# yumi-crew/pose_estimation

Hardware: NVIDIA B200
Metric: icp_hypotheses_per_s (higher is better)
Workload: dtype f32

## Files before the change

### pose_estimation_b200/csrc/icp.cu

```cuda
#include <algorithm>

#include "block_select.cuh"
#include "nn_cache.cuh"
#include "nn_graph.cuh"
#include "nn_search.cuh"
#include "nn_upfront.cuh"

namespace peb {

namespace {

constexpr int kIcpThreads = 128;
constexpr int kMinBlocksSingle = 5;
#ifndef PEB_MIN_BLOCKS_BATCH
#define PEB_MIN_BLOCKS_BATCH 8
#endif
constexpr int kMinBlocksBatch = PEB_MIN_BLOCKS_BATCH;
#ifndef PEB_MIN_BLOCKS_SEARCH
#define PEB_MIN_BLOCKS_SEARCH 10
#endif
constexpr int kMinBlocksSearch = PEB_MIN_BLOCKS_SEARCH;

struct IcpLaunch {
  GridView grid;
// ... 111 lines not shown
    sm[warp][lane] = v;
  }
  __syncthreads();
  if (threadIdx.x < NACC) {
    double r = 0.0;
#pragma unroll
    for (int w = 0; w < kW; ++w) r += sm[w][threadIdx.x];
    sm_out[threadIdx.x] = r;
  }
  __syncthreads();
}

__global__ void __launch_bounds__(128) icp_anchor_kernel(const IcpLaunch L, int* __restrict__ anchors) {
  const int a = blockIdx.x * blockDim.x + threadIdx.x;
  const int h = blockIdx.y;
  if (a >= L.n_anchor) return;
  const IcpState* st = L.states + h;
  float T[16];
  bool apply = false;
#pragma unroll
  for (int i = 0; i < 16; ++i) {
    T[i] = __ldcg(&st->final_t.m[i]);
    if (T[i] != ((i % 5 == 0) ? 1.0f : 0.0f)) apply = true;
  }
  float4 p = L.src[32 * a];
  if (apply) {
    float ox, oy, oz;
    transform_icp(T, p.x, p.y, p.z, ox, oy, oz);
    p.x = ox;
    p.y = oy;
    p.z = oz;
  }
  const NnBest best = grid_nn<1, true>(L.grid, p.x, p.y, p.z, L.stop_d2);
  anchors[static_cast<size_t>(h) * L.n_anchor + a] = best.j;
}

__device__ __forceinline__ unsigned long long global_ns() {
  unsigned long long t;
  asm volatile("mov.u64 %0, %%globaltimer;" : "=l"(t));
  return t;
}

template <int MB>
__device__ __noinline__ void finish_iteration(IcpState* st, const IcpCriteria* cr, const double* acc, Mat4* trace,
                                              int trace_cap, unsigned long long* dbg) {
  if (dbg) dbg[5] = global_ns();
  IcpState s = *st;
  if (dbg) dbg[6] = global_ns() + (s.iterations < -5 ? 1 : 0);
  icp_finish_iteration(s, *cr, acc);
  if (dbg) dbg[7] = global_ns() + (s.iterations < -5 ? 1 : 0);
  s.ticket = 0;
  if (trace && s.state != PEB_NO_CORRESPONDENCES && s.iterations >= 1 && s.iterations <= trace_cap)
    trace[s.iterations - 1] = s.inc;
  *st = s;
}

__device__ __forceinline__ void pdl_trigger_and_wait() {
  asm volatile("griddepcontrol.launch_dependents;");
  asm volatile("griddepcontrol.wait;" ::: "memory");
}

__device__ __forceinline__ int ld_acquire_gpu(const int* p) {
  int v;
  asm volatile("ld.acquire.gpu.global.s32 %0, [%1];" : "=r"(v) : "l"(p) : "memory");
  return v;
}


constexpr int kEpochStopped = 1 << 20;
constexpr unsigned long long kFlagWaitLimitNs = 20ull * 1000ull * 1000ull * 1000ull;
__device__ __forceinline__ void wait_for_hypothesis(const int* __restrict__ solved, int need, int* err_flag) {
  if (threadIdx.x == 0 && ld_acquire_gpu(solved) < need) {
    const unsigned long long t0 = global_ns();
    unsigned spins = 0;
    while (ld_acquire_gpu(solved) < need) {
      __nanosleep(40);
      if ((++spins & 0xFFFu) == 0u && global_ns() - t0 > kFlagWaitLimitNs) {
        atomicExch(err_flag, 1);
        break;
      }
    }
  }
  __syncthreads();
}

__device__ __forceinline__ void wait_for_search(const int* __restrict__ searched, int need, const int* __restrict__ solved,
                                                int* err_flag) {
  if (threadIdx.x == 0 && ld_acquire_gpu(searched) < need && ld_acquire_gpu(solved) < kEpochStopped) {
    const unsigned long long t0 = global_ns();
    unsigned spins = 0;
    while (ld_acquire_gpu(searched) < need && ld_acquire_gpu(solved) < kEpochStopped) {
      __nanosleep(40);
      if ((++spins & 0xFFFu) == 0u && global_ns() - t0 > kFlagWaitLimitNs) {
        atomicExch(err_flag, 1);
        break;
      }
    }
  }
  __syncthreads();
}

__device__ __forceinline__ bool graph_pays(const IcpLaunch& L, const IcpState* st) {
  if (!L.knn) return false;
  if (L.knn_kappa <= 0.0f) return true;
  const double mse = __ldcg(&st->cur_mse);
  const double cnt = __ldcg(L.knn_stat + 1);
  return cnt > 0.0 && 4.0 * mse * static_cast<double>(L.knn_kappa) * cnt < __ldcg(L.knn_stat);
}

template <int EST, int NACC>
__device__ __forceinline__ void accumulate_pair_impl(const GridView& g, const float4& p, const NnBest& best,
                                                     double (&acc)[NACC]) {
  const float4 t = g.pts[best.j];
  if (EST == PEB_ESTIMATOR_SVD) {
    const double sx = p.x, sy = p.y, sz = p.z, tx = t.x, ty = t.y, tz = t.z;
    acc[0] += 1.0;
    acc[1] += sx;
    acc[2] += sy;
    acc[3] += sz;
    acc[4] += tx;
    acc[5] += ty;
    acc[6] += tz;
    acc[7] = fma(tx, sx, acc[7]);
    acc[8] = fma(tx, sy, acc[8]);
    acc[9] = fma(tx, sz, acc[9]);
    acc[10] = fma(ty, sx, acc[10]);
    acc[11] = fma(ty, sy, acc[11]);
    acc[12] = fma(ty, sz, acc[12]);
    acc[13] = fma(tz, sx, acc[13]);
    acc[14] = fma(tz, sy, acc[14]);
    acc[15] = fma(tz, sz, acc[15]);
    acc[16] += static_cast<double>(best.d2);
  } else {
    acc[0] += 1.0;
    acc[NACC - 1] += static_cast<double>(best.d2);
    const float4 nr = g.normals[best.j];
    if (finite3(t.x, t.y, t.z) && finite3(nr.x, nr.y, nr.z)) {
      const float sx = p.x, sy = p.y, sz = p.z, dx = t.x, dy = t.y, dz = t.z;
      const float nx = nr.x, ny = nr.y, nz = nr.z;
      const double a = nz * sy - ny * sz;
      const double b = nx * sz - nz * sx;
      const double c = ny * sx - nx * sy;
      acc[1] += a * a;
      acc[2] += a * b;
      acc[3] += a * c;
      acc[4] += a * nx;
      acc[5] += a * ny;
      acc[6] += a * nz;
      acc[7] += b * b;
      acc[8] += b * c;
      acc[9] += b * nx;
      acc[10] += b * ny;
      acc[11] += b * nz;
      acc[12] += c * c;
      acc[13] += c * nx;
      acc[14] += c * ny;
      acc[15] += c * nz;
      acc[16] += nx * nx;
      acc[17] += nx * ny;
      acc[18] += nx * nz;
      acc[19] += ny * ny;
      acc[20] += ny * nz;
      acc[21] += nz * nz;
      const double d = nx * dx + ny * dy + nz * dz - nx * sx - ny * sy - nz * sz;
      acc[22] += a * d;
      acc[23] += b * d;
      acc[24] += c * d;
      acc[25] += nx * d;
      acc[26] += ny * d;
      acc[27] += nz * d;
    }
  }
}
template <int EST, int NACC>
__device__ __forceinline__ void accumulate_pair(const GridView& g, const float4& p, const NnBest& best,
                                                double (&acc)[NACC]) {
  static_assert((EST == PEB_ESTIMATOR_SVD && NACC == kAccSvd) || (EST != PEB_ESTIMATOR_SVD && NACC == kAccLls), "layout");
  accumulate_pair_impl<EST, NACC>(g, p, best, acc);
}

__device__ __forceinline__ NnBest first_iteration_search(const IcpLaunch& L, int h, int i, bool valid, const float4& p,
                                                         const float* T, bool apply, CoopTile* tile) {
  NnBest best;
  best.d2 = pos_inf();
  best.idx = -1;
  best.j = -1;
  bool need = false;
  int group = 0;
  if (valid) {
    int j_seed = -1;
    float4 a = make_float4(0.f, 0.f, 0.f, 0.f);
    group = 0;
    const int patch = i >> 5;
#pragma unroll 1
    for (int k = 0; k < 2 && j_seed < 0; ++k) {
      const int pa = patch + k;
      if (pa >= L.n_anchor) break;
      const int js = __ldcg(L.anchors + static_cast<size_t>(h) * L.n_anchor + pa);
      if (js < 0) continue;
      a = L.src[32 * pa];
      if (apply) {
        float ox, oy, oz;
        transform_icp(T, a.x, a.y, a.z, ox, oy, oz);
        a.x = ox;
        a.y = oy;
        a.z = oz;
      }
      const float ax = p.x - a.x, ay = p.y - a.y, az = p.z - a.z;
      if (ax * ax + ay * ay + az * az <= L.seed_guard2 * L.grid.h * L.grid.h) {
        j_seed = js;
        group = k;
      }
    }
    if (j_seed >= 0) {
      best = (L.knn && L.cold_graph) ? grid_nn_graph_descend(L.grid, L.knn, p.x, p.y, p.z, j_seed)
                                     : grid_nn_seed_probe(L.grid, p.x, p.y, p.z, j_seed, a.x, a.y, a.z);
      need = true;
    } else {
      best = grid_nn<1>(L.grid, p.x, p.y, p.z, L.stop_d2);
      PEB_COOP_COUNT_LANE(6);
    }
  }
  PEB_COOP_COUNT(7, __any_sync(0xFFFFFFFFu, valid && !need) ? 1 : 0);
#pragma unroll 1
  for (int k = 0; k < 2; ++k) {
    const bool mine = need && group == k;
    bool done = false;
    if (L.coop_max_rows > 0) done = grid_nn_coop_verify(L.grid, tile, mine, p.x, p.y, p.z, L.stop_d2, L.coop_max_rows, best);
    if (!done && mine) grid_ball_search(L.grid, p.x, p.y, p.z, L.stop_d2, best);
  }
  return best;
}

template <int G, int EST, bool CERT, int UPF, int NACC>
__device__ __forceinline__ void icp_query(const IcpLaunch& L, const int h, float4* __restrict__ work, const int i,
                                          const bool first, const bool apply, const bool graph, const float* T,
                                          CoopTile* tile, double (&acc)[NACC]) {
  const int lane_in_group = threadIdx.x & (G - 1);
  const bool in = i < L.n_src;
  float4 p = make_float4(0.f, 0.f, 0.f, 1.f);
  if (in) p = first ? L.src[i] : work[i];
  const int j_prev = first ? -1 : __float_as_int(p.w);
  const bool valid = in && finite3(p.x, p.y, p.z);
  float moved = 0.0f;
  if (valid && apply) {
    float ox, oy, oz;
    transform_icp(T, p.x, p.y, p.z, ox, oy, oz);
    if (CERT) {
      const float mx = ox - p.x, my = oy - p.y, mz = oz - p.z;
      moved = sqrtf(mx * mx + my * my + mz * mz);
    }
    p.x = ox;
    p.y = oy;
    p.z = oz;
  }
  NnBest best;
  best.d2 = pos_inf();
  best.idx = -1;
  best.j = -1;
  float slack = -1.0f;
  if (G == 1 && first && L.anchors) {
    best = first_iteration_search(L, h, i, valid, p, T, apply, tile);
    if (CERT && valid) L.slack[static_cast<size_t>(h) * L.n_src + i] = -1.0f;
  } else if (valid) {
    float* sl = L.slack + static_cast<size_t>(h) * L.n_src + i;
    if (G == 1 && L.warm && j_prev >= 0 && j_prev < L.grid.n) {
      if (CERT) {
        slack = *sl - 2.000002f * moved - 1e-5f * L.grid.h;
        if (slack > 0.0f) {
          const float4 t = L.grid.pts[j_prev];
          best.d2 = l2_simple(p.x, p.y, p.z, t.x, t.y, t.z);
          best.idx = __float_as_int(t.w);
          best.j = j_prev;
        } else {
          best = grid_nn_warm_cert(L.grid, p.x, p.y, p.z, j_prev, L.stop_d2, L.margin, &slack);
        }
        *sl = slack;
      } else {
        if (UPF == 4 || UPF == 6) best = graph ? grid_nn_warm_graph(L.grid, L.knn, p.x, p.y, p.z, j_prev, L.stop_d2, kGraphSkipHopeless, L.launch_idx <= L.knn_peek_until, UPF == 6 ? L.knn_aux : nullptr)
                                   : grid_nn_warm(L.grid, p.x, p.y, p.z, j_prev, L.stop_d2);
        else best = UPF ? grid_nn_warm_upfront<(UPF == 3 ? 3 : 2)>(L.grid, p.x, p.y, p.z, j_prev, L.stop_d2)
                        : grid_nn_warm(L.grid, p.x, p.y, p.z, j_prev, L.stop_d2);
      }
    } else {
      best = grid_nn<G>(L.grid, p.x, p.y, p.z, L.stop_d2);
      if (CERT && lane_in_group == 0) *sl = -1.0f;
    }
  }
  if (in && lane_in_group == 0 && (first || valid)) {
    p.w = __int_as_float(best.j);
    work[i] = p;
  }
  bool keep = valid && best.idx >= 0;
  if (keep && static_cast<double>(best.d2) > L.max_dist_sqr) keep = false;
  if (keep && L.use_rejector && !(best.d2 < L.rej_max2)) keep = false;
  if (in && lane_in_group == 0 && L.corr_idx) {
    const int orig = __float_as_int(L.src[i].w);
    L.corr_idx[orig] = keep ? best.idx : -1;
    L.corr_d2[orig] = keep ? best.d2 : 0.0f;
  }
  if (keep && lane_in_group == 0) accumulate_pair<EST>(L.grid, p, best, acc);
}

template <int UPF>
__device__ __forceinline__ NnBest icp_search_query(const IcpLaunch& L, const int h, float4* __restrict__ work, const int i,
                                                   const bool first, const bool apply, const bool graph, const float* T,
                                                   CoopTile* tile, float4& p, bool& valid) {
  const bool in = i < L.n_src;
  p = make_float4(0.f, 0.f, 0.f, 1.f);
  if (in) p = first ? L.src[i] : work[i];
  const int j_prev = first ? -1 : __float_as_int(p.w);
  valid = in && finite3(p.x, p.y, p.z);
  if (valid && apply) {
    float ox, oy, oz;
    transform_icp(T, p.x, p.y, p.z, ox, oy, oz);
    p.x = ox;
    p.y = oy;
    p.z = oz;
  }
  NnBest best;
  best.d2 = pos_inf();
  best.idx = -1;
  best.j = -1;
  if (first && L.anchors) {
    best = first_iteration_search(L, h, i, valid, p, T, apply, tile);
  } else if (valid) {
    if (L.warm && j_prev >= 0 && j_prev < L.grid.n) {
      if (UPF == 4 || UPF == 6) best = graph ? grid_nn_warm_graph(L.grid, L.knn, p.x, p.y, p.z, j_prev, L.stop_d2, kGraphSkipHopeless, L.launch_idx <= L.knn_peek_until, UPF == 6 ? L.knn_aux : nullptr)
                                 : grid_nn_warm(L.grid, p.x, p.y, p.z, j_prev, L.stop_d2);
      else best = grid_nn_warm(L.grid, p.x, p.y, p.z, j_prev, L.stop_d2);
    } else {
      best = grid_nn<1>(L.grid, p.x, p.y, p.z, L.stop_d2);
    }
  }
  if (in && (first || valid)) {
    p.w = __int_as_float(best.j);
    work[i] = p;
  }
  return best;
}

__device__ __forceinline__ bool keep_pair(const IcpLaunch& L, const bool valid, const NnBest& best) {
  bool keep = valid && best.idx >= 0;
  if (keep && static_cast<double>(best.d2) > L.max_dist_sqr) keep = false;
  if (keep && L.use_rejector && !(best.d2 < L.rej_max2)) keep = false;
  return keep;
}

template <bool FIRST, int UPF>
__device__ __forceinline__ void load_launch_flags(const IcpLaunch& L, const IcpState* st, float* s_inc, int* s_flags) {
  if (threadIdx.x < 16) s_inc[threadIdx.x] = FIRST ? __ldcg(&st->final_t.m[threadIdx.x]) : __ldcg(&st->inc.m[threadIdx.x]);
  if (threadIdx.x == 32) {
    const int active = __ldcg(&st->active);
    const int first = FIRST ? 1 : 0;
    int apply = 1;
    if (first) {
      apply = 0;
      for (int i = 0; i < 16; ++i) {
        const float g = __ldcg(&st->final_t.m[i]);
        if (g != ((i % 5 == 0) ? 1.0f : 0.0f)) apply = 1;
      }
    }
    s_flags[0] = active;
    s_flags[1] = first;
    s_flags[2] = apply;
    const int graph = ((UPF == 4 || UPF == 6) && graph_pays(L, st)) ? 1 : 0;
    s_flags[3] = graph;
  }
}

template <int G, int EST, int MB, bool CERT, bool FIRST, int UPF>
__device__ __forceinline__ void icp_iteration_body(const IcpLaunch& L, const int h, const int blk) {
  unsigned long long t_dbg[5];
  if (L.dbg) t_dbg[0] = global_ns();
  constexpr int NACC = (EST == PEB_ESTIMATOR_SVD) ? kAccSvd : kAccLls;
  __shared__ double sm[kIcpThreads / 32][kAccMax];
  __shared__ double sm_tot[kAccMax];
  __shared__ float s_inc[16];
  __shared__ int s_flags[4];
  __shared__ CoopTile s_tile[kIcpThreads / 32];
  IcpState* st = L.states + h;
  if (threadIdx.x < 16) s_inc[threadIdx.x] = FIRST ? __ldcg(&st->final_t.m[threadIdx.x]) : __ldcg(&st->inc.m[threadIdx.x]);
  if (threadIdx.x == 32) {
    const int active = __ldcg(&st->active);
    const int first = FIRST ? 1 : 0;
    int apply = 1;
    if (first) {
      apply = 0;
      for (int i = 0; i < 16; ++i) {
        const float g = __ldcg(&st->final_t.m[i]);
        if (g != ((i % 5 == 0) ? 1.0f : 0.0f)) apply = 1;
      }
    }
    s_flags[0] = active;
    s_flags[1] = first;
    s_flags[2] = apply;
    const int graph = ((UPF == 4 || UPF == 6) && graph_pays(L, st)) ? 1 : 0;
    s_flags[3] = graph;
  }
  __syncthreads();
  if (!s_flags[0]) return;
  constexpr bool first = FIRST;
  const bool apply = s_flags[2] != 0;
  const float* T = s_inc;

  double acc[NACC];
#pragma unroll
  for (int i = 0; i < NACC; ++i) acc[i] = 0.0;

  float4* work = L.work + static_cast<size_t>(h) * L.n_src;
  constexpr int kQ = kIcpThreads / G;
  const int q_local = threadIdx.x / G;
  const bool graph = (UPF == 4 || UPF == 6) && s_flags[3] != 0;
  for (int base = blk * kQ; base < L.n_src; base += L.blocks_per_hyp * kQ)
    icp_query<G, EST, CERT, UPF>(L, h, work, base + q_local, first, apply, graph, T, &s_tile[threadIdx.x >> 5], acc);

  if (L.dbg) t_dbg[1] = global_ns();
  const double r = block_reduce_acc<NACC>(acc, sm);
  double* part = L.partials + (static_cast<size_t>(h) * L.part_stride) * kAccMax;
  if (threadIdx.x < NACC) __stcg(part + static_cast<size_t>(blk) * kAccMax + threadIdx.x, r);
  __threadfence();
  __syncthreads();
  __shared__ int s_last;
  if (threadIdx.x == 0) {
    const unsigned t = atomicAdd(&st->ticket, 1u);
    s_last = (t == static_cast<unsigned>(L.blocks_per_hyp) - 1u);
  }
  __syncthreads();
  if (!s_last) return;
  __threadfence();
  if (L.dbg) t_dbg[2] = global_ns();
  reduce_partials<NACC>(part, L.blocks_per_hyp, sm, sm_tot);
  if (L.dbg) t_dbg[3] = global_ns();
  if (threadIdx.x == 0) {
    finish_iteration<MB>(st, &L.crit, sm_tot, L.trace, L.trace_cap, (L.dbg && h == 0) ? L.dbg + 8 * L.launch_idx : nullptr);
    if (L.dbg && h == 0) {
      t_dbg[4] = global_ns();
      for (int k = 0; k < 5; ++k) L.dbg[8 * L.launch_idx + k] = t_dbg[k];
    }
    if (L.epochs) {
      const int still_active = st->active;
      __threadfence();
      atomicAdd(L.epochs + h, still_active ? 1 : kEpochStopped);
    }
  }
}

template <int G, int EST, int MB, bool CERT, bool FIRST, int UPF = 0>
__global__ void __launch_bounds__(kIcpThreads, MB) icp_iteration_kernel(const IcpLaunch L) {
  if (FIRST || L.epochs == nullptr) {
    pdl_trigger_and_wait();
  } else {
    asm volatile("griddepcontrol.launch_dependents;");
    wait_for_hypothesis(L.epochs + blockIdx.y, L.launch_idx, L.err_flag);
  }
  icp_iteration_body<G, EST, MB, CERT, FIRST, UPF>(L, blockIdx.y, blockIdx.x);
}

template <int MB, bool FIRST, int UPF>
__global__ void __launch_bounds__(kIcpThreads, MB) icp_search_kernel(const IcpLaunch L) {
  if (FIRST || L.epochs == nullptr) {
    pdl_trigger_and_wait();
  } else {
    asm volatile("griddepcontrol.launch_dependents;");
    wait_for_hypothesis(L.epochs + blockIdx.y, L.launch_idx, L.err_flag);
  }
  const int h = blockIdx.y, blk = blockIdx.x;
  __shared__ float s_inc[16];
  __shared__ int s_flags[4];
  __shared__ CoopTile s_tile[kIcpThreads / 32];
  IcpState* st = L.states + h;
  load_launch_flags<FIRST, UPF>(L, st, s_inc, s_flags);
  __syncthreads();
  if (s_flags[0]) {
    const bool apply = s_flags[2] != 0;
    const bool graph = (UPF == 4 || UPF == 6) && s_flags[3] != 0;
    float4* work = L.work + static_cast<size_t>(h) * L.n_src;
    for (int base = blk * kIcpThreads; base < L.n_src; base += gridDim.x * kIcpThreads) {
      const int i = base + threadIdx.x;
      float4 p;
      bool valid;
      const NnBest best = icp_search_query<UPF>(L, h, work, i, FIRST, apply, graph, s_inc, &s_tile[threadIdx.x >> 5], p, valid);
      int* w = reinterpret_cast<int*>(work + i) + 3;
      if (valid && best.j >= 0 && !finite3(p.x, p.y, p.z)) *w = -2 - best.j;
      else if (!FIRST && !valid && i < L.n_src && __float_as_int(p.w) <= -2) *w = -1;
    }
  }
  if (L.epochs && s_flags[0]) {
    __syncthreads();
    if (threadIdx.x == 0) {
      __threadfence();
      if (atomicAdd(&st->ticket_search, 1u) == gridDim.x - 1u) {
        st->ticket_search = 0u;
        __threadfence();
        atomicAdd(&st->searched, 1);
      }
    }
  }
}

template <int EST, int MB, bool CHAIN>
__global__ void __launch_bounds__(kIcpThreads, MB) icp_moment_kernel(const IcpLaunch L, const unsigned char* __restrict__ kept) {
  if (L.epochs == nullptr) {
    pdl_trigger_and_wait();
  } else {
    asm volatile("griddepcontrol.launch_dependents;");
    wait_for_search(&L.states[blockIdx.y].searched, L.launch_idx + 1, L.epochs + blockIdx.y, L.err_flag);
  }
  const int h = blockIdx.y, blk = blockIdx.x;
  constexpr int NACC = (EST == PEB_ESTIMATOR_SVD) ? kAccSvd : kAccLls;
  __shared__ double sm[kIcpThreads / 32][kAccMax];
  __shared__ double sm_tot[kAccMax];
  __shared__ int s_active;
  IcpState* st = L.states + h;
  if (threadIdx.x == 0) s_active = __ldcg(&st->active);
  __syncthreads();
  if (!s_active) return;

  double acc[NACC];
#pragma unroll
  for (int i = 0; i < NACC; ++i) acc[i] = 0.0;
  const float4* work = L.work + static_cast<size_t>(h) * L.n_src;
  for (int i = blk * kIcpThreads + threadIdx.x; i < L.n_src; i += L.blocks_per_hyp * kIcpThreads) {
    const float4 p = __ldcg(work + i);
    bool valid = finite3(p.x, p.y, p.z);
    int j = __float_as_int(p.w);
    if (j <= -2) {
      valid = true;
      j = -2 - j;
    }
    if (CHAIN) {
      NnBest best;
      const bool keep = valid && j >= 0 && kept[static_cast<size_t>(h) * L.n_src + i];
      if (keep) {
        const float4 t = L.grid.pts[j];
        best.d2 = l2_simple(p.x, p.y, p.z, t.x, t.y, t.z);
        best.idx = point_index(t);
        best.j = j;
        accumulate_pair<EST>(L.grid, p, best, acc);
      }
      if (L.corr_idx) {
        const int orig = __float_as_int(L.src[i].w);
        L.corr_idx[orig] = keep ? best.idx : -1;
        L.corr_d2[orig] = keep ? best.d2 : 0.0f;
      }
      continue;
    }
    if (!valid || j < 0) continue;
    const float4 t = L.grid.pts[j];
    NnBest best;
    best.d2 = l2_simple(p.x, p.y, p.z, t.x, t.y, t.z);
    best.idx = point_index(t);
    best.j = j;
    if (keep_pair(L, valid, best)) accumulate_pair<EST>(L.grid, p, best, acc);
  }

  const double r = block_reduce_acc<NACC>(acc, sm);
  double* part = L.partials + (static_cast<size_t>(h) * L.part_stride) * kAccMax;
  if (threadIdx.x < NACC) __stcg(part + static_cast<size_t>(blk) * kAccMax + threadIdx.x, r);
  __threadfence();
  __syncthreads();
  __shared__ int s_last;
  if (threadIdx.x == 0) {
    const unsigned t = atomicAdd(&st->ticket, 1u);
    s_last = (t == static_cast<unsigned>(L.blocks_per_hyp) - 1u);
  }
  __syncthreads();
  if (!s_last) return;
  __threadfence();
  reduce_partials<NACC>(part, L.blocks_per_hyp, sm, sm_tot);
  if (threadIdx.x == 0) {
    finish_iteration<MB>(st, &L.crit, sm_tot, L.trace, L.trace_cap, nullptr);
    if (L.epochs) {
      const int still_active = st->active;
      __threadfence();
      atomicAdd(L.epochs + h, still_active ? 1 : kEpochStopped);
    }
  }
}

constexpr int kRejThreads = 1024;

struct RejChain {
  int kind[PEB_MAX_REJECTORS];
  int min_corr[PEB_MAX_REJECTORS];
  double value[PEB_MAX_REJECTORS];
  int n;
  unsigned char* kept;
  unsigned long long* o2o;
};

__device__ __forceinline__ NnBest rej_pair(const IcpLaunch& L, const float4* __restrict__ work, int i, float4& p, bool& valid) {
  p = __ldcg(work + i);
  valid = finite3(p.x, p.y, p.z);
  int j = __float_as_int(p.w);
  if (j <= -2) {
    valid = true;
    j = -2 - j;
  }
  NnBest best;
  best.d2 = pos_inf();
  best.idx = -1;
  best.j = -1;
  if (valid && j >= 0) {
    const float4 t = L.grid.pts[j];
    best.d2 = l2_simple(p.x, p.y, p.z, t.x, t.y, t.z);
    best.idx = point_index(t);
    best.j = j;
  }
  return best;
}

__device__ __forceinline__ unsigned abs_bits(float v) { return __float_as_uint(v) & 0x7FFFFFFFu; }

__device__ __forceinline__ float rej_score(const IcpLaunch& L, const float4& p, int j) {
  const float4 t = L.grid.pts[j];
  const float dx = p.x - t.x, dy = p.y - t.y, dz = p.z - t.z;
  return __fadd_rn(__fadd_rn(__fmul_rn(dx, dx), __fmul_rn(dz, dz)), __fmul_rn(dy, dy));
}

__device__ __forceinline__ int rej_count(const unsigned char* kept, int n) {
  int m = 0;
  for (int base = 0; base < n; base += kRejThreads) {
    const int i = base + threadIdx.x;
    m += __syncthreads_count(i < n && kept[i]);
  }
  return m;
}

__global__ void __launch_bounds__(kRejThreads, 1) icp_reject_kernel(const IcpLaunch L, const RejChain R) {
  pdl_trigger_and_wait();
  __shared__ unsigned hist[2048];
  __shared__ unsigned s_state[2];
  __shared__ unsigned s_wsum[32];
  __shared__ int s_active;
  const int h = blockIdx.x;
  if (threadIdx.x == 0) s_active = __ldcg(&L.states[h].active);
  __syncthreads();
  if (!s_active) return;
  const int n = L.n_src;
  const float4* work = L.work + static_cast<size_t>(h) * n;
  unsigned char* kept = R.kept + static_cast<size_t>(h) * n;
  unsigned long long* tab = R.o2o ? R.o2o + static_cast<size_t>(h) * L.grid.n : nullptr;
  for (int i = threadIdx.x; i < n; i += kRejThreads) {
    float4 p;
    bool valid;
    const NnBest b = rej_pair(L, work, i, p, valid);
    kept[i] = keep_pair(L, valid, b) ? 1 : 0;
  }
  __syncthreads();
  for (int s = 0; s < R.n; ++s) {
    const int kind = R.kind[s];
    if (kind == PEB_REJECTOR_DISTANCE) {
      const float lim = static_cast<float>(R.value[s] * R.value[s]);
      for (int i = threadIdx.x; i < n; i += kRejThreads) {
        if (!kept[i]) continue;
        float4 p;
        bool valid;
        const NnBest b = rej_pair(L, work, i, p, valid);
        if (!(b.d2 < lim)) kept[i] = 0;
      }
    } else if (kind == PEB_REJECTOR_MEDIAN_DISTANCE) {
      const int m = rej_count(kept, n);
      if (m == 0) continue;
      auto score = [&](int i) {
        if (!kept[i]) return -1.0f;
        float4 p;
        bool valid;
        const NnBest b = rej_pair(L, work, i, p, valid);
        return __uint_as_float(abs_bits(rej_score(L, p, b.j)));
      };
      const float med = block_select_nth<decltype(score), true>(score, n, m / 2, hist, s_state, s_wsum);
      const double lim = static_cast<double>(med) * R.value[s];
      for (int i = threadIdx.x; i < n; i += kRejThreads) {
        if (!kept[i]) continue;
        float4 p;
        bool valid;
        const NnBest b = rej_pair(L, work, i, p, valid);
        if (!(static_cast<double>(rej_score(L, p, b.j)) <= lim)) kept[i] = 0;
      }
    } else if (kind == PEB_REJECTOR_ONE_TO_ONE) {
      for (int i = threadIdx.x; i < n; i += kRejThreads) {
        if (!kept[i]) continue;
        float4 p;
        bool valid;
        const NnBest b = rej_pair(L, work, i, p, valid);
        const unsigned long long key = (static_cast<unsigned long long>(abs_bits(b.d2)) << 32) |
                                       static_cast<unsigned>(__float_as_int(L.src[i].w));
        atomicMin(tab + b.j, key);
      }
      __syncthreads();
      for (int i = threadIdx.x; i < n; i += kRejThreads) {
        if (!kept[i]) continue;
        float4 p;
        bool valid;
        const NnBest b = rej_pair(L, work, i, p, valid);
        const unsigned long long key = (static_cast<unsigned long long>(abs_bits(b.d2)) << 32) |
                                       static_cast<unsigned>(__float_as_int(L.src[i].w));
        if (__ldcg(tab + b.j) == key) __stcg(tab + b.j, ~0ull);
        else kept[i] = 0;
      }
    } else {
      const int m = rej_count(kept, n);
      const float ratio = fminf(1.0f, fmaxf(0.0f, static_cast<float>(R.value[s])));
      const int n_keep = max(static_cast<int>(floorf(ratio * static_cast<float>(m))), R.min_corr[s]);
      if (n_keep >= m) continue;
      unsigned vb = 0u;
      int o_cut = -1;
      if (n_keep > 0) {
        auto d2_of = [&](int i) {
          if (!kept[i]) return -1.0f;
          float4 p;
          bool valid;
          return __uint_as_float(abs_bits(rej_pair(L, work, i, p, valid).d2));
        };
        vb = __float_as_uint(block_select_nth<decltype(d2_of), true>(d2_of, n, n_keep - 1, hist, s_state, s_wsum));
        int below = 0;
        for (int base = 0; base < n; base += kRejThreads) {
          const int i = base + threadIdx.x;
          bool lt = false;
          if (i < n && kept[i]) {
            float4 p;
            bool valid;
            lt = abs_bits(rej_pair(L, work, i, p, valid).d2) < vb;
          }
          below += __syncthreads_count(lt);
        }
        auto src_at_cut = [&](int i) {
          if (!kept[i]) return -1.0f;
          float4 p;
          bool valid;
          if (abs_bits(rej_pair(L, work, i, p, valid).d2) != vb) return -1.0f;
          return __int_as_float(__float_as_int(L.src[i].w));
        };
        o_cut = __float_as_int(block_select_nth<decltype(src_at_cut), true>(src_at_cut, n, n_keep - below - 1, hist, s_state, s_wsum));
      }
      for (int i = threadIdx.x; i < n; i += kRejThreads) {
        if (!kept[i]) continue;
        bool stay = false;
        if (n_keep > 0) {
          float4 p;
          bool valid;
          const unsigned db = abs_bits(rej_pair(L, work, i, p, valid).d2);
          stay = db < vb || (db == vb && __float_as_int(L.src[i].w) <= o_cut);
        }
        if (!stay) kept[i] = 0;
      }
    }
    __syncthreads();
  }
}

constexpr int kBinQ = 4;
constexpr int kBinTile = kBinQ * kIcpThreads;
constexpr int kBinClasses = 5;

__device__ __forceinline__ int bin_class_of_rows(int rows) {
  return rows >= 7 ? 0 : rows >= 5 ? 1 : rows >= 3 ? 2 : rows == 2 ? 3 : 4;
}

template <int EST, int MB>
__global__ void __launch_bounds__(kIcpThreads, MB) icp_iteration_binned_kernel(const IcpLaunch L) {
  if (L.epochs == nullptr) {
    pdl_trigger_and_wait();
  } else {
    asm volatile("griddepcontrol.launch_dependents;");
    wait_for_hypothesis(L.epochs + blockIdx.y, L.launch_idx, L.err_flag);
  }
  const int h = blockIdx.y, blk = blockIdx.x;
  constexpr int NACC = (EST == PEB_ESTIMATOR_SVD) ? kAccSvd : kAccLls;
  __shared__ double sm[kIcpThreads / 32][kAccMax];
  __shared__ double sm_tot[kAccMax];
  __shared__ float s_inc[16];
  __shared__ int s_active;
  __shared__ float s_qx[kBinTile], s_qy[kBinTile], s_qz[kBinTile], s_d2[kBinTile];
  __shared__ int s_idx[kBinTile], s_j[kBinTile];
  __shared__ unsigned short s_key[kBinTile], s_perm[kBinTile];
  __shared__ int s_cnt[2][kBinClasses + 1];
  IcpState* st = L.states + h;
  if (threadIdx.x < 16) s_inc[threadIdx.x] = __ldcg(&st->inc.m[threadIdx.x]);
  if (threadIdx.x == 32) s_active = __ldcg(&st->active);
  if (threadIdx.x >= 64 && threadIdx.x < 64 + 2 * (kBinClasses + 1)) (&s_cnt[0][0])[threadIdx.x - 64] = 0;
  __syncthreads();
  if (!s_active) return;
  const float* T = s_inc;
// ... 1070 lines not shown
```

Before: 17810.

## Compact graph-search fallbacks into per-warp queues to cut divergence

In the search kernel's graph-warm path, each thread first tries a cheap k-NN graph lookup. Queries that still need a full grid ball search are compacted through a per-warp shared-memory queue and drained 32 at a time, so the expensive search runs with full warps instead of diverged lanes. This adds shared-memory queue traffic, ballot/popc bookkeeping and a dependence on new helpers (grid_nn_graph_try, grid_ball_search). It also drops the UPF template from the scalar query path.

```diff
diff --git a/pose_estimation_b200/csrc/icp.cu b/pose_estimation_b200/csrc/icp.cu
--- a/pose_estimation_b200/csrc/icp.cu
+++ b/pose_estimation_b200/csrc/icp.cu
@@ -437,10 +437,9 @@
   if (keep && lane_in_group == 0) accumulate_pair<EST>(L.grid, p, best, acc);
 }
 
-template <int UPF>
 __device__ __forceinline__ NnBest icp_search_query(const IcpLaunch& L, const int h, float4* __restrict__ work, const int i,
-                                                   const bool first, const bool apply, const bool graph, const float* T,
-                                                   CoopTile* tile, float4& p, bool& valid) {
+                                                   const bool first, const bool apply, const float* T, CoopTile* tile,
+                                                   float4& p, bool& valid) {
   const bool in = i < L.n_src;
   p = make_float4(0.f, 0.f, 0.f, 1.f);
   if (in) p = first ? L.src[i] : work[i];
@@ -460,13 +459,8 @@
   if (first && L.anchors) {
     best = first_iteration_search(L, h, i, valid, p, T, apply, tile);
   } else if (valid) {
-    if (L.warm && j_prev >= 0 && j_prev < L.grid.n) {
-      if (UPF == 4 || UPF == 6) best = graph ? grid_nn_warm_graph(L.grid, L.knn, p.x, p.y, p.z, j_prev, L.stop_d2, kGraphSkipHopeless, L.launch_idx <= L.knn_peek_until, UPF == 6 ? L.knn_aux : nullptr)
-                                 : grid_nn_warm(L.grid, p.x, p.y, p.z, j_prev, L.stop_d2);
-      else best = grid_nn_warm(L.grid, p.x, p.y, p.z, j_prev, L.stop_d2);
-    } else {
-      best = grid_nn<1>(L.grid, p.x, p.y, p.z, L.stop_d2);
-    }
+    if (L.warm && j_prev >= 0 && j_prev < L.grid.n) best = grid_nn_warm(L.grid, p.x, p.y, p.z, j_prev, L.stop_d2);
+    else best = grid_nn<1>(L.grid, p.x, p.y, p.z, L.stop_d2);
   }
   if (in && (first || valid)) {
     p.w = __int_as_float(best.j);
@@ -592,6 +586,82 @@
   icp_iteration_body<G, EST, MB, CERT, FIRST, UPF>(L, blockIdx.y, blockIdx.x);
 }
 
+
+__device__ __forceinline__ int search_slot(float x, float y, float z, int j) {
+  return (j >= 0 && !finite3(x, y, z)) ? -2 - j : j;
+}
+
+struct SearchQueued {
+  float x, y, z;
+  int cand;
+  int i;
+};
+constexpr int kSearchQueue = 64;
+
+template <int UPF>
+__device__ __forceinline__ void icp_search_graph_queued(const IcpLaunch& L, float4* __restrict__ work, const bool apply,
+                                                        const float* T) {
+  __shared__ SearchQueued s_queue[kIcpThreads / 32][kSearchQueue];
+  SearchQueued* queue = s_queue[threadIdx.x >> 5];
+  const int lane = threadIdx.x & 31;
+  const bool peek = L.launch_idx <= L.knn_peek_until;
+  int n_queue = 0;
+  auto drain = [&](int count) {
+    if (lane < count) {
+      const SearchQueued e = queue[n_queue - count + lane];
+      NnBest best;
+      if (e.cand >= 0) {
+        const float4 t = L.grid.pts[e.cand];
+        best.d2 = l2_simple(e.x, e.y, e.z, t.x, t.y, t.z);
+        best.idx = point_index(t);
+        best.j = e.cand;
+        grid_ball_search(L.grid, e.x, e.y, e.z, L.stop_d2, best);
+      } else {
+        best = grid_nn<1>(L.grid, e.x, e.y, e.z, L.stop_d2);
+      }
+      work[e.i] = make_float4(e.x, e.y, e.z, __int_as_float(search_slot(e.x, e.y, e.z, best.j)));
+    }
+    n_queue -= count;
+    __syncwarp();
+  };
+  for (int base = blockIdx.x * kIcpThreads; base < L.n_src; base += gridDim.x * kIcpThreads) {
+    const int i = base + threadIdx.x;
+    const bool in = i < L.n_src;
+    float4 p = make_float4(0.f, 0.f, 0.f, 1.f);
+    if (in) p = work[i];
+    const int j_prev = __float_as_int(p.w);
+    bool need = false;
+    int cand = -1;
+    if (in && finite3(p.x, p.y, p.z)) {
+      if (apply) {
+        float ox, oy, oz;
+        transform_icp(T, p.x, p.y, p.z, ox, oy, oz);
+        p.x = ox;
+        p.y = oy;
+        p.z = oz;
+      }
+      need = true;
+      if (L.warm && j_prev >= 0 && j_prev < L.grid.n) {
+        NnBest best;
+        need = !grid_nn_graph_try(L.grid, L.knn, p.x, p.y, p.z, j_prev, best, kGraphSkipHopeless, peek,
+                                  UPF == 6 ? L.knn_aux : nullptr);
+        if (need) cand = best.j;
+        else work[i] = make_float4(p.x, p.y, p.z, __int_as_float(search_slot(p.x, p.y, p.z, best.j)));
+      }
+    } else if (in && j_prev <= -2) {
+      reinterpret_cast<int*>(work + i)[3] = -1;
+    }
+    const unsigned m = __ballot_sync(0xFFFFFFFFu, need);
+    if (m) {
+      if (need) queue[n_queue + __popc(m & ((1u << lane) - 1u))] = SearchQueued{p.x, p.y, p.z, cand, i};
+      n_queue += __popc(m);
+      __syncwarp();
+      if (n_queue >= 32) drain(32);
+    }
+  }
+  if (n_queue) drain(n_queue);
+}
+
 template <int MB, bool FIRST, int UPF>
 __global__ void __launch_bounds__(kIcpThreads, MB) icp_search_kernel(const IcpLaunch L) {
   if (FIRST || L.epochs == nullptr) {
@@ -611,11 +681,12 @@
     const bool apply = s_flags[2] != 0;
     const bool graph = (UPF == 4 || UPF == 6) && s_flags[3] != 0;
     float4* work = L.work + static_cast<size_t>(h) * L.n_src;
-    for (int base = blk * kIcpThreads; base < L.n_src; base += gridDim.x * kIcpThreads) {
+    if (!FIRST && graph) icp_search_graph_queued<UPF>(L, work, apply, s_inc);
+    else for (int base = blk * kIcpThreads; base < L.n_src; base += gridDim.x * kIcpThreads) {
       const int i = base + threadIdx.x;
       float4 p;
       bool valid;
-      const NnBest best = icp_search_query<UPF>(L, h, work, i, FIRST, apply, graph, s_inc, &s_tile[threadIdx.x >> 5], p, valid);
+      const NnBest best = icp_search_query(L, h, work, i, FIRST, apply, s_inc, &s_tile[threadIdx.x >> 5], p, valid);
       int* w = reinterpret_cast<int*>(work + i) + 3;
       if (valid && best.j >= 0 && !finite3(p.x, p.y, p.z)) *w = -2 - best.j;
       else if (!FIRST && !valid && i < L.n_src && __float_as_int(p.w) <= -2) *w = -1;
```

Result: faster. 19100, median of 6 (+7.2%).
